# KC-decoder/Multimodal-Brain-Pattern-Identification_XAI

Measured on AMD Instinct MI355X. Metric: samples/sec train (multimodal SpectrogramCNN+EEGNet fusion, B=64/GPU, 4x128x256 spectro + 10000x19 EEG), higher is better.
Workload: dtype bf16

## Files before the change

include/brainxai.h:

```cpp
#ifndef BRAINXAI_H
#define BRAINXAI_H

#include <stddef.h>
#include <stdint.h>

#ifdef __cplusplus
extern "C" {
#endif

#define BX_VERSION 100

enum { BX_F32 = 0, BX_BF16 = 1 };
enum { BX_POOL_MAX = 0, BX_POOL_AVG = 1 };
enum { BX_OK = 0, BX_EINVAL = -1, BX_EDTYPE = -2, BX_EALIGN = -3, BX_EWORKSPACE = -4, BX_EHIP = -5,
       BX_EUNSUPPORTED = -6 };
enum { BX_ALGO_AUTO = 0, BX_ALGO_DIRECT = 1, BX_ALGO_MFMA = 2 };
enum { BX_EPI_RELU = 1, BX_EPI_MASK_BITS = 2 };

typedef void* bxStream;

int bx_version(void);
const char* bx_last_error_string(void);

int bx_nchw_to_nhwc(const float* src, void* dst, int B, int C, int H, int W, int Cp, int dtype, bxStream stream);
// ... 10 lines not shown
  void* packed_mfma;
  int Cout, Cin, I_p, O_p, transpose_flip, block_begin;
} bxPackJob;
int bx_conv3x3_pack_many(const bxPackJob* jobs_device, int njobs, int total_blocks, bxStream stream);
int bx_conv3x3_pack_many_layout(const bxPackJob* jobs_device, int njobs, int total_blocks, const float* src_nchw,
                                void* dst_nhwc_bf16, int B, int C, int H, int W, int Cp, bxStream stream);
int bx_conv3x3_pack_layout_ex(const bxPackJob* jobs_device, int njobs, int total_blocks, const float* src_nchw,
                              const float* const* src_slot, void* dst_nhwc_bf16, int B, int C, int H, int W, int Cp, bxStream stream);
int bx_conv3x3_pack_many_step(const bxPackJob* jobs_device, int njobs, int total_blocks, const float* src_nchw,
                              void* dst_nhwc_bf16, int B, int C, int H, int W, int Cp, uint64_t* state_a, uint64_t* out_a,
                              uint64_t* state_b, uint64_t* out_b, bxStream stream);
int bx_conv3x3_pair_supported(int C0_p, int C1, int C2, int dtype);
int bx_conv3x3_pair(const void* x, const void* packed1_mfma, const float* bias1, const void* packed2_mfma, const float* bias2,
                    void* y1, void* y2, unsigned char* mask1, unsigned char* mask2, int B, int H, int W, int C0_p, int C1, int C2,
                    int dtype, bxStream stream);
int bx_conv3x3(const void* x, const float* packed_f32, const void* packed_mfma, const float* bias,
               const void* relu_mask_src, const void* addend, void* y,
               int B, int H, int W, int Ci, int Co, int dtype, int flags, int algo, bxStream stream);
size_t bx_conv3x3_wgrad_workspace(int B, int H, int W, int Ci_p, int Co, int dtype, int algo);
int bx_conv3x3_wgrad(const void* x, const void* dz, float* dw_oihw, float* dbias, int B, int H, int W,
                     int Cin, int Ci_p, int Co, int dtype, int algo, void* workspace, size_t workspace_bytes,
                     bxStream stream);
typedef struct {
  const void* partial; float* dw; float* db;
  int nsplit, Cin, Co, ma, nb, ztiles, nfrag4, valid;
} bxWgradPending;
int bx_conv3x3_wgrad_chained(const void* x, const void* dz, float* dw_oihw, float* dbias, int B, int H, int W, int Cin,
                             int Ci_p, int Co, int dtype, int algo, void* workspace, size_t workspace_bytes,
                             bxWgradPending* pending, bxStream stream);
int bx_conv3x3_wgrad_finish(bxWgradPending* pending, bxStream stream);
int bx_conv3x3_carry(const void* x, const float* packed_f32, const void* packed_mfma, const float* bias,
                     const void* relu_mask_src, const void* addend, void* y, int B, int H, int W, int Ci, int Co,
                     int dtype, int flags, int algo, bxWgradPending* pending, bxStream stream);

int bx_profile_next_conv3(void* ev_start, void* ev_stop);

typedef struct {
  int B, H, W;
  int Cin_p;
  int C;
  int pool;
  int training;
  float eps, momentum;
  float dropout_p;
  uint32_t salt;
  int dtype;
  uint32_t* sync;
  void* route;
} bxTailDesc;
size_t bx_block_tail_route_bytes(const bxTailDesc* d);
#define BX_TAIL_SYNC_WORDS 8192
#define BX_TAIL_SYNC_FWD 0
#define BX_TAIL_SYNC_BWD 4096
size_t bx_block_tail_workspace(const bxTailDesc* d);
int bx_block_tail_fwd(const bxTailDesc* d, const void* y3, const void* x, const float* w1x1, int Cin,
                      const float* b1x1, const float* bn_weight, const float* bn_bias,
                      float* running_mean, float* running_var, int64_t* num_batches_tracked,
                      const uint64_t* seed, void* pooled, void* out, float* save_mean, float* save_invstd,
                      void* workspace, size_t workspace_bytes, bxStream stream);
int bx_set_tree_max_rows(int rows);
int bx_set_tail_fold(int mask);
int bx_block_conv3_tail_fwd(const bxTailDesc* d, const void* y2, const void* w3_mfma, const float* b3, void* y3,
                            const void* x, const float* w1x1, int Cin, const float* b1x1, const float* bn_weight,
                            const float* bn_bias, float* running_mean, float* running_var, int64_t* num_batches_tracked,
                            const uint64_t* seed, void* pooled, void* out, float* save_mean, float* save_invstd,
                            void* workspace, size_t workspace_bytes, bxStream stream);
// ... 171 lines not shown
```

multimodal-brain-pattern-identification_xai_amd/_lib.py:

```python
from __future__ import annotations

import ctypes as C
import os

HERE = os.path.dirname(os.path.abspath(__file__))
LIB_PATH = os.path.join(HERE, "libbrainxai.so")

BX_F32, BX_BF16 = 0, 1
BX_POOL_MAX, BX_POOL_AVG = 0, 1
BX_ALGO_AUTO, BX_ALGO_DIRECT, BX_ALGO_MFMA = 0, 1, 2
BX_EPI_RELU = 1
BX_EPI_MASK_BITS = 2
BX_TAIL_SYNC_WORDS = 8192
BX_EEG_CAM_CONV1, BX_EEG_CAM_DEPTHWISE, BX_EEG_CAM_SEPARABLE = 0, 1, 2

vp, i32, i64, u32, f32, sz = C.c_void_p, C.c_int, C.c_int64, C.c_uint32, C.c_float, C.c_size_t


class TailDesc(C.Structure):
    _fields_ = [("B", i32), ("H", i32), ("W", i32), ("Cin_p", i32), ("C", i32), ("pool", i32), ("training", i32),
                ("eps", f32), ("momentum", f32), ("dropout_p", f32), ("salt", u32), ("dtype", i32), ("sync", vp), ("route", vp)]


class EegDesc(C.Structure):
# ... 29 lines not shown
class PackJob(C.Structure):
    _fields_ = [("w_oihw", vp), ("packed_mfma", vp), ("Cout", i32), ("Cin", i32), ("I_p", i32), ("O_p", i32),
                ("transpose_flip", i32), ("block_begin", i32)]


class EegGrads(C.Structure):
    _fields_ = [(n, vp) for n in ("conv1_w", "bn1_w", "bn1_b", "dw_w", "bn2_w", "bn2_b", "sep_w", "bn3_w", "bn3_b")]


P = C.POINTER
SIGNATURES = {
    "bx_version": (i32, []),
    "bx_last_error_string": (C.c_char_p, []),
    "bx_nchw_to_nhwc": (i32, [vp, vp, i32, i32, i32, i32, i32, i32, vp]),
    "bx_nhwc_to_nchw": (i32, [vp, vp, i32, i32, i32, i32, i32, i32, vp]),
    "bx_conv3x3_pack": (i32, [vp, vp, vp, i32, i32, i32, i32, i32, vp]),
    "bx_conv3x3_packed_mfma_bytes": (sz, [i32, i32]),
    "bx_conv3x3_packed_split_bytes": (sz, [i32, i32]),
    "bx_conv3x3_pack_split": (i32, [vp, vp, i32, i32, i32, i32, i32, vp]),
    "bx_conv3x3_pack_many": (i32, [vp, i32, i32, vp]),
    "bx_conv3x3_pack_many_layout": (i32, [vp, i32, i32, vp, vp, i32, i32, i32, i32, i32, vp]),
    "bx_conv3x3_pack_layout_ex": (i32, [vp, i32, i32, vp, vp, vp, i32, i32, i32, i32, i32, vp]),
    "bx_conv3x3_pair_supported": (i32, [i32, i32, i32, i32]),
    "bx_conv3x3_pair": (i32, [vp] * 9 + [i32] * 7 + [vp]),
    "bx_conv3x3_pack_many_step": (i32, [vp, i32, i32, vp, vp, i32, i32, i32, i32, i32, vp, vp, vp, vp, vp]),
    "bx_scale_dev": (i32, [vp, vp, vp, sz, vp]),
    "bx_abs": (i32, [vp, vp, sz, vp]),
    "bx_conv3x3": (i32, [vp, vp, vp, vp, vp, vp, vp, i32, i32, i32, i32, i32, i32, i32, i32, vp]),
    "bx_conv3x3_carry": (i32, [vp, vp, vp, vp, vp, vp, vp, i32, i32, i32, i32, i32, i32, i32, i32, P(WgradPending), vp]),
    "bx_conv3x3_wgrad_workspace": (sz, [i32, i32, i32, i32, i32, i32, i32]),
    "bx_conv3x3_wgrad": (i32, [vp, vp, vp, vp, i32, i32, i32, i32, i32, i32, i32, i32, vp, sz, vp]),
    "bx_conv3x3_wgrad_chained": (i32, [vp, vp, vp, vp, i32, i32, i32, i32, i32, i32, i32, i32, vp, sz, P(WgradPending), vp]),
    "bx_conv3x3_wgrad_finish": (i32, [P(WgradPending), vp]),
    "bx_block_tail_workspace": (sz, [P(TailDesc)]),
    "bx_block_tail_fwd": (i32, [P(TailDesc), vp, vp, vp, i32, vp, vp, vp, vp, vp, vp, vp, vp, vp, vp, vp, vp, sz, vp]),
    "bx_set_tree_max_rows": (i32, [i32]),
    "bx_set_tail_fold": (i32, [i32]),
    "bx_block_tail_route_bytes": (sz, [vp]),
    "bx_block_conv3_tail_fwd": (i32, [P(TailDesc), vp, vp, vp, vp, vp, vp, i32, vp, vp, vp, vp, vp, vp, vp, vp, vp, vp, vp, vp, sz, vp]),
    "bx_block_tail_bwd": (i32, [P(TailDesc), vp, vp, vp, vp, vp, i32, vp, vp, vp, vp, vp, vp, vp, vp, vp, vp, vp, sz, vp]),
    "bx_relu": (i32, [vp, vp, sz, i32, vp]),
    "bx_gap_fc_lsm_fwd": (i32, [vp, vp, vp, vp, vp, i32, i32, i32, i32, i32, vp]),
    "bx_gap_fc_lsm_bwd": (i32, [vp, vp, vp, vp, vp, vp, vp, i32, i32, i32, i32, i32, vp]),
    "bx_linear_lsm_fwd": (i32, [vp, vp, vp, vp, i32, i32, i32, vp]),
    "bx_linear_lsm_bwd": (i32, [vp, vp, vp, vp, vp, vp, vp, i32, i32, i32, vp]),
    "bx_fusion_head_fwd": (i32, [vp, vp, vp, vp, vp, vp, vp, vp, i32, i32, i32, vp]),
    "bx_fusion_head_bwd": (i32, [vp] * 13 + [i32, i32, i32, vp]),
    "bx_mm_head_workspace": (sz, [i32, i32, i32]),
    "bx_mm_head_fwd": (i32, [vp] * 15 + [i32] * 7 + [vp]),
    "bx_mm_head_bwd": (i32, [vp] * 22 + [sz] + [i32] * 7 + [vp]),
    "bx_kldiv_fwd_bwd": (i32, [vp, vp, vp, vp, i32, i32, i32, f32, vp]),
    "bx_eeg_saved_bytes": (sz, [P(EegDesc)]),
    "bx_eeg_workspace": (sz, [P(EegDesc)]),
    "bx_eeg_features_fwd": (i32, [P(EegDesc), P(EegParams), vp, vp, vp, vp, vp, sz, vp]),
    "bx_eeg_features_bwd": (i32, [P(EegDesc), P(EegParams), vp, vp, vp, vp, P(EegGrads), vp, vp, sz, vp]),
    "bx_eeg_saved_layout": (i32, [P(EegDesc), P(sz), P(sz)]),
    "bx_eeg_gradcam_workspace": (sz, [P(EegDesc), i32, i32]),
    "bx_eeg_gradcam": (i32, [P(EegDesc), P(EegParams), vp, vp, vp, i32, i32, i32, vp, vp, vp, vp, sz, vp]),
    "bx_eeg_deep_saved_bytes": (sz, [P(EegDeepDesc)]),
    "bx_eeg_deep_workspace": (sz, [P(EegDeepDesc)]),
    "bx_eeg_deep_fwd": (i32, [P(EegDeepDesc), P(EegDeepParams), vp, vp, vp, vp, vp, vp, sz, vp]),
    "bx_eeg_deep_bwd": (i32, [P(EegDeepDesc), P(EegDeepParams), vp, vp, vp, vp, vp, P(EegDeepGrads), vp, vp, sz, vp]),
    "bx_attention_workspace": (sz, [i32]),
    "bx_attention_fwd": (i32, [vp] * 10 + [i32, i32, i32, vp]),
    "bx_attention_bwd": (i32, [vp] * 16 + [sz, i32, i32, i32, vp]),
    "bx_gradcam_reduce": (i32, [vp, vp, vp, vp, i32, i32, i32, i32, i32, i32, vp]),
# ... 58 lines not shown
```

multimodal-brain-pattern-identification_xai_amd/csrc/conv3x3_mfma.hip:

```cpp
#include <stdlib.h>
#include "bx_common.h"
#include <string.h>

typedef __attribute__((ext_vector_type(8))) short bf16x8;
typedef __attribute__((ext_vector_type(4))) float f32x4;
typedef unsigned int u32x4 __attribute__((ext_vector_type(4)));
typedef unsigned int u32x2 __attribute__((ext_vector_type(2)));

static inline int mfma_ck(int Ci) { return Ci < 64 ? Ci : 64; }
static inline int mfma_ks(int ck) { return (9 * ck + 31) / 32; }

int bx_conv3x3_mfma_supported(int Ci, int Co, int dtype) {
  if (dtype != BX_BF16) return 0;
  if (!(Ci == 8 || Ci == 16 || Ci == 32 || (Ci >= 64 && Ci % 64 == 0))) return 0;
  return (Co >= 16 && Co % 16 == 0) || (Co == 8 && (Ci == 16 || Ci == 32));
}
static inline int mfma_ow(int O_p) { return O_p < 16 ? 16 : O_p; }
extern "C" size_t bx_conv3x3_packed_mfma_bytes(int I_p, int O_p) {
  if (!bx_conv3x3_mfma_supported(I_p, O_p, BX_BF16)) return 0;
  const int ck = mfma_ck(I_p);
  return (size_t)(I_p / ck) * mfma_ks(ck) * mfma_ow(O_p) * 32 * sizeof(bf16_t);
}

__global__ void k_pack_mfma(const float* __restrict__ w, bf16_t* __restrict__ wp, int Cout, int Cin, int I_p, int O_p, int tf,
// ... 1416 lines not shown
      const float4 v3 = *reinterpret_cast<const float4*>(src + (size_t)(c + 3 * S) * per_split);
      s.x += v0.x; s.y += v0.y; s.z += v0.z; s.w += v0.w;
      s.x += v1.x; s.y += v1.y; s.z += v1.z; s.w += v1.w;
      s.x += v2.x; s.y += v2.y; s.z += v2.z; s.w += v2.w;
      s.x += v3.x; s.y += v3.y; s.z += v3.z; s.w += v3.w;
    }
    for (; c < nsplit; c += S) {
      const float4 v = *reinterpret_cast<const float4*>(src + (size_t)c * per_split);
      s.x += v.x; s.y += v.y; s.z += v.z; s.w += v.w;
    }
  }
  sm[threadIdx.x] = s;
  __syncthreads();
  if (part == 0 && live) {
    float4 r = sm[o];
    for (int k = 1; k < S; ++k) { const float4 v = sm[k * NO + o]; r.x += v.x; r.y += v.y; r.z += v.z; r.w += v.w; }
    const float rr[4] = {r.x, r.y, r.z, r.w};
    if (e4 < (size_t)nfrag4) {
      const int NT = 9 * MA * NB;
      const int lane = (int)(e4 & 63), tl = (int)(e4 >> 6);
      const int i = tl % NT, yz = tl / NT, z = yz % ztiles, y = yz / ztiles;
      const int n = i % NB, m = (i / NB) % MA, t = i / (NB * MA);
      const int cout = (z * NB + n) * 16 + (lane & 15), cin0 = (y * MA + m) * 16 + 4 * (lane >> 4);
#pragma unroll
      for (int j = 0; j < 4; ++j)
        if (cin0 + j < Cin) dw[((size_t)cout * Cin + cin0 + j) * 9 + t] = rr[j];
    } else if (db) {
      const size_t b0 = (e4 - nfrag4) * 4;
#pragma unroll
      for (int j = 0; j < 4; ++j) db[b0 + j] = rr[j];
    }
  }
}
__global__ __launch_bounds__(256) void k_wgrad_reduce3(WgradRedJob jb) {
  __shared__ float4 sm[256];
  wgrad_reduce3_body(jb, blockIdx.x, sm);
}

typedef __attribute__((ext_vector_type(4))) short s16x4;
typedef __attribute__((address_space(3))) s16x4 lds_s16x4;

__device__ __forceinline__ bf16x8 tr_read8(const char* lds, int off0, int off1) {
  const s16x4 lo = __builtin_amdgcn_ds_read_tr16_b64_v4i16((lds_s16x4*)(lds + off0));
  const s16x4 hi = __builtin_amdgcn_ds_read_tr16_b64_v4i16((lds_s16x4*)(lds + off1));
  return (bf16x8){lo[0], lo[1], lo[2], lo[3], hi[0], hi[1], hi[2], hi[3]};
}

template <int MA, int NB, int TW>
__global__ __launch_bounds__(256, 2) void k_wgrad_mfma(const bf16_t* __restrict__ x, const bf16_t* __restrict__ dz, float* __restrict__ partial,
    int H, int W, int Ci_p, int Co, int tiles_x, int tiles_y, int ntiles, int tiles_per_split, WgradRedJob prev, int zextra) {
  constexpr int TH = 8, HWID = TW + 2, HH = TH + 2, CIT = 16 * MA, COT = 16 * NB, XB = CIT * 2, ZB = COT * 2;
  constexpr int KPW = TH * TW / 32 / 4;
  constexpr int XS_BYTES = HH * HWID * XB;
  extern __shared__ __attribute__((aligned(16))) char lds[];
  if ((int)blockIdx.z < zextra) {
    const int rid = ((int)blockIdx.z * (int)gridDim.y + (int)blockIdx.y) * (int)gridDim.x + (int)blockIdx.x;
    if (rid < prev.nblocks) wgrad_reduce3_body(prev, rid, reinterpret_cast<float4*>(lds));
    return;
  }
  const int bz = (int)blockIdx.z - zextra, gz = (int)gridDim.z - zextra;
  char* xs = lds;
  char* zs = lds + XS_BYTES;
  const int wave = threadIdx.x >> 6, lane = threadIdx.x & 63, g = lane >> 4, li = lane & 15;
  const int q = li >> 2, pc = li & 3;
  const int ci0 = blockIdx.y * CIT, co0 = bz * COT;
  const bool want_bias = blockIdx.y == 0;

  f32x4 acc[9][MA][NB];
#pragma unroll
// ... 342 lines not shown
}
int bx_wgrad_mfma_supported(int Ci_p, int Co, int dtype) {
  return dtype == BX_BF16 && Ci_p % 8 == 0 && Co % 16 == 0 && (Co < 32 || Co % 32 == 0) && (Ci_p < 32 || Ci_p % 32 == 0);
}
size_t bx_wgrad_mfma_workspace(int B, int H, int W, int Ci_p, int Co) {
  const WgradPlan p = wgrad_plan(B, H, W, Ci_p, Co);
  return (size_t)p.nsplit * ((size_t)p.ytiles * p.ztiles * 9 * p.ma * p.nb * 256 + Co) * sizeof(float);
}
template <int MA, int NB, int TW>
static void launch_wgrad(const WgradPlan& p, const void* x, const void* dz, float* ws, int H, int W, int Ci_p, int Co, const WgradRedJob& prev,
                         int zextra, hipStream_t s) {
  dim3 grid(p.nsplit, p.ytiles, p.ztiles + zextra);
  hipLaunchKernelGGL((k_wgrad_mfma<MA, NB, TW>), grid, dim3(256), p.lds, s, (const bf16_t*)x, (const bf16_t*)dz, ws, H, W, Ci_p, Co,
                     p.tiles_x, p.tiles_y, p.ntiles, p.tps, prev, zextra);
}
static int wgrad_reduce_slices(size_t per_split, int nsplit, bool chained) {
  if (!chained) return per_split >= 65536 ? 4 : per_split >= 8192 ? 16 : 64;
  int S = 1;
  while (S < 64 && nsplit > 8 * S) S *= 2;
  return S;
}
static WgradRedJob wgrad_job_from(const bxWgradPending* pd, bool chained) {
  WgradRedJob jb;
  jb.partial = (const float*)pd->partial; jb.dw = pd->dw; jb.db = pd->db; jb.nsplit = pd->nsplit; jb.Cin = pd->Cin; jb.Co = pd->Co;
  jb.MA = pd->ma; jb.NB = pd->nb; jb.ztiles = pd->ztiles; jb.nfrag4 = pd->nfrag4;
  const size_t per_split = (size_t)pd->nfrag4 * 4 + pd->Co;
  jb.S = wgrad_reduce_slices(per_split, pd->nsplit, chained);
  const int per_wg = 256 / jb.S;
  jb.nblocks = (int)((per_split / 4 + per_wg - 1) / per_wg);
  return jb;
}
int bx_wgrad_mfma_finish(bxWgradPending* pd, hipStream_t s) {
  if (!pd || !pd->valid) return BX_OK;
  const WgradRedJob jb = wgrad_job_from(pd, false);
  hipLaunchKernelGGL(k_wgrad_reduce3, dim3(jb.nblocks), dim3(256), 0, s, jb);
  pd->valid = 0;
  BX_CHECK_LAUNCH("bx_conv3x3_wgrad(mfma reduce)");
  return BX_OK;
}
int bx_wgrad_mfma_launch(const void* x, const void* dz, float* dw, float* db, int B, int H, int W, int Cin, int Ci_p,
                         int Co, void* ws, size_t ws_bytes, bxWgradPending* pending, hipStream_t s) {
  const WgradPlan p = wgrad_plan(B, H, W, Ci_p, Co);
  (void)ws_bytes;
  BX_REQUIRE((size_t)B * H * W * (Ci_p > Co ? Ci_p : Co) * 2 < ((size_t)1 << 31), "bx_conv3x3_wgrad(mfma): an activation tensor of 2 GiB or more is not supported");
  BX_REQUIRE(!pending || !pending->valid || pending->partial != ws, "bx_conv3x3_wgrad(chained): the pending partials live in this call's workspace");
  float* part = (float*)ws;
  WgradRedJob prev;
  memset(&prev, 0, sizeof(prev));
  int zextra = 0;
  if (pending && pending->valid) {
    prev = wgrad_job_from(pending, true);
    zextra = (prev.nblocks + p.nsplit * p.ytiles - 1) / (p.nsplit * p.ytiles);
  }
  if (p.ma == 2 && p.nb == 2) {
    const int nred = pending && pending->valid ? (prev.nblocks + 7) / 8 * 8 : 0;
    const int ranges8 = (p.nsplit + 7) / 8;
    const int nwg = nred + ranges8 * 8 * p.ytiles * p.ztiles;
    const size_t lds = (size_t)10 * (p.tw + 2) * 64 + (size_t)8 * p.tw * 64 + 256;
    if (p.tw == 16)
      hipLaunchKernelGGL((k_wgrad_own<16, 2>), dim3(nwg), dim3(256), lds, s, (const bf16_t*)x, (const bf16_t*)dz, part, H, W, Ci_p, Co,
                         p.tiles_x, p.tiles_y, p.ntiles, p.tps, p.nsplit, p.ytiles, p.ztiles, prev, nred);
    else
      hipLaunchKernelGGL((k_wgrad_own<32, 2>), dim3(nwg), dim3(256), lds, s, (const bf16_t*)x, (const bf16_t*)dz, part, H, W, Ci_p, Co,
                         p.tiles_x, p.tiles_y, p.ntiles, p.tps, p.nsplit, p.ytiles, p.ztiles, prev, nred);
  } else {
#define BX_WG(MA_, NB_) do { if (p.tw == 16) launch_wgrad<MA_, NB_, 16>(p, x, dz, part, H, W, Ci_p, Co, prev, zextra, s); \
                             else launch_wgrad<MA_, NB_, 32>(p, x, dz, part, H, W, Ci_p, Co, prev, zextra, s); } while (0)
    if (p.ma == 1 && p.nb == 1) BX_WG(1, 1);
    else if (p.ma == 1) BX_WG(1, 2);
    else BX_WG(2, 1);
#undef BX_WG
  }
  BX_CHECK_LAUNCH("bx_conv3x3_wgrad(mfma)");
  bxWgradPending cur;
  cur.partial = part; cur.dw = dw; cur.db = db; cur.nsplit = p.nsplit; cur.Cin = Cin; cur.Co = Co; cur.ma = p.ma; cur.nb = p.nb;
  cur.ztiles = p.ztiles; cur.nfrag4 = p.ytiles * p.ztiles * 9 * p.ma * p.nb * 64; cur.valid = 1;
  if (pending) { *pending = cur; return BX_OK; }
  return bx_wgrad_mfma_finish(&cur, s);
}
```

multimodal-brain-pattern-identification_xai_amd/ops.py:

```python
from __future__ import annotations

import ctypes as C
from types import SimpleNamespace

import torch

from . import _lib as L

CONV_ALGO = L.BX_ALGO_AUTO
WGRAD_ALGO = L.BX_ALGO_AUTO
CONV_PROFILE = None
import os as _os
OVERLAP_EEG = int(_os.environ.get("BX_OVERLAP_EEG", "1"))
OVERLAP_EEG_DDP = _os.environ.get("BX_OVERLAP_EEG_DDP", "0") == "1"


def overlap_eeg_now() -> bool:
    if CONV_PROFILE is not None or not (OVERLAP_EEG >= 2 or (OVERLAP_EEG == 1 and torch.cuda.is_current_stream_capturing())):
        return False
    import torch.distributed as dist
    return OVERLAP_EEG_DDP or not (dist.is_available() and dist.is_initialized())


def fork_eeg(device, *read_on_side):
# ... 405 lines not shown
def _wgrad(x, dz, w: torch.Tensor, b: torch.Tensor, chain: bool = False):
    lib = L.load()
    B, H, W, Cip = x.shape
    Co = dz.shape[3]
    dt = bx_dtype(x.dtype)
    algo = WGRAD_ALGO
    need = lib.bx_conv3x3_wgrad_workspace(B, H, W, Cip, Co, dt, algo)
    dw, db = new_grad(w), new_grad(b)
    if chain and WGRAD_CHAIN and algo != L.BX_ALGO_DIRECT:
        st = _wg_chain_state(x.device)
        if st.pend.valid and st.stream != _stream():
            wgrad_flush(x.device)
        buf = st.ring[st.slot]
        if buf is None or buf.numel() < need:
            if buf is not None:
                st.retired.append(buf)
            big = max([int(need), 1 << 20] + [b.numel() for b in st.ring if b is not None])
            buf = torch.empty(big, dtype=torch.uint8, device=x.device)
            st.ring[st.slot] = buf
        st.stream = _stream()
        with _Timed("wgrad", ("conv", B, H, W, Cip, Co)):
            L.check(lib.bx_conv3x3_wgrad_chained(_p(x), _p(dz), _p(dw), _p(db), B, H, W, w.shape[1], Cip, Co, dt, algo, _p(buf), buf.numel(),
                                                 C.byref(st.pend), st.stream), "bx_conv3x3_wgrad_chained")
        st.keep = (buf, dw, db)
        st.slot ^= 1
        return dw, db
    ws = workspace(need, x.device)
    with _Timed("wgrad", ("conv", B, H, W, Cip, Co)):
        L.check(lib.bx_conv3x3_wgrad(_p(x), _p(dz), _p(dw), _p(db), B, H, W, w.shape[1], Cip, Co, dt, algo, _p(ws), ws.numel(), _stream()),
                "bx_conv3x3_wgrad")
    return dw, db


def _tail_desc(x, shape, dt, cfg, route=None) -> L.TailDesc:
    B, H, W, Cc = shape
    return L.TailDesc(B, H, W, x.shape[3], Cc, L.BX_POOL_MAX if cfg.pool == "max" else L.BX_POOL_AVG, 1 if cfg.training else 0,
                      cfg.eps, cfg.momentum, float(cfg.dropout_p), cfg.salt, bx_dtype(dt), _p(cfg.sync), _p(route))


class BlockFn(torch.autograd.Function):

    @staticmethod
    def forward(ctx, x, w1, b1, w2, b2, w3, b3, bnw, bnb, w11, b11, rm, rv, nbt, cfg):
        lib = L.load()
        dt = x.dtype
        ws_, bs_ = (w1, w2, w3), (b1, b2, b3)
        acts, pre = [x], None
        B, H, W, _ = x.shape
        Cc = w3.shape[0]
        fused = FUSE_POOL and dt == torch.bfloat16 and CONV_ALGO != L.BX_ALGO_DIRECT and cfg.preact != 3 and Cc >= 16
        packed3 = None
        first = 0
        masks = None
        if (CONV_PAIR and dt == torch.bfloat16 and CONV_ALGO != L.BX_ALGO_DIRECT and cfg.preact not in (1, 2)
                and lib.bx_conv3x3_pair_supported(x.shape[3], w1.shape[0], w2.shape[0], bx_dtype(dt))):
            pk = []
            for k in range(2):
                packed = cfg.prepacked.get(cfg.pack_base + k, False) if cfg.prepacked is not None else None
                pk.append(packed if packed is not None else _pack(ws_[k], flip=False, dtype=dt))
            if pk[0][1] is not None and pk[1][1] is not None:
                need_y1 = cfg.keep is not None or (getattr(cfg, "grad_mode", True) and any(ctx.needs_input_grad[:11]))
                y1 = torch.empty(B, H, W, w1.shape[0], dtype=dt, device=x.device) if need_y1 else None
                y2 = torch.empty(B, H, W, w2.shape[0], dtype=dt, device=x.device)
                if need_y1 and MASK_BITS and w1.shape[0] <= 32:
                    masks = (torch.empty(B, H, W, w1.shape[0] // 4, dtype=torch.uint8, device=x.device),
                             torch.empty(B, H, W, w2.shape[0] // 4, dtype=torch.uint8, device=x.device))
                with _Timed("fwd", ("pair", B, H, W, x.shape[3], (w1.shape[0], w2.shape[0]))):
                    L.check(lib.bx_conv3x3_pair(_p(x), _p(pk[0][1]), _p(b1), _p(pk[1][1]), _p(b2), _p(y1), _p(y2),
                                                _p(masks[0]) if masks else None, _p(masks[1]) if masks else None, B, H, W, x.shape[3],
                                                w1.shape[0], w2.shape[0], bx_dtype(dt), _stream()), "bx_conv3x3_pair")
                acts += [y1 if y1 is not None else x.new_empty(0), y2]
                first = 2
        for k in range(first, 3):
            packed = cfg.prepacked.get(cfg.pack_base + k, False) if cfg.prepacked is not None else None
            if packed is None:
                packed = _pack(ws_[k], flip=False, dtype=dt)
            if k == 2 and fused and packed[1] is not None:
                packed3 = packed
                break
            if cfg.preact == k + 1:
                pre = _conv(acts[-1], packed, bs_[k], None, None, False, dt)
                y = torch.empty_like(pre)
                L.check(lib.bx_relu(_p(pre), _p(y), pre.numel(), bx_dtype(dt), _stream()), "bx_relu")
            else:
                y = _conv(acts[-1], packed, bs_[k], None, None, True, dt)
            acts.append(y)
        seed = None
        if cfg.training and cfg.dropout_p > 0:
            seed = cfg.seed if cfg.seed is not None else next_seed(x.device)
        pooled = torch.empty(B, H // 2, W // 2, Cc, dtype=dt, device=x.device)
        out = torch.empty_like(pooled)
        mean = torch.empty(Cc, dtype=torch.float32, device=x.device)
        invstd = torch.empty_like(mean)
        route = None
        if packed3 is not None:
            need_bwd = getattr(cfg, "grad_mode", True) and any(ctx.needs_input_grad[:11])
            use_route = TAIL_ROUTE and cfg.keep is None
            y3 = torch.empty(B, H, W, Cc, dtype=dt, device=x.device) if (cfg.keep is not None or (need_bwd and not use_route)) else None
            if need_bwd and use_route:
                route = torch.empty(B * (H // 2) * (W // 2) * Cc // 2, dtype=torch.uint8, device=x.device)
            desc = _tail_desc(x, (B, H, W, Cc), dt, cfg, route)
            ws = workspace(lib.bx_block_tail_workspace(C.byref(desc)), x.device)
            if CONV_PROFILE is not None:
                pe0, pe1 = torch.cuda.Event(enable_timing=True), torch.cuda.Event(enable_timing=True)
                pe0.record(); pe1.record()
                L.check(lib.bx_profile_next_conv3(pe0.cuda_event, pe1.cuda_event), "bx_profile_next_conv3")
                CONV_PROFILE.append(("fwd", pe0, pe1, ("conv3+pool", B, H, W, acts[2].shape[3], Cc)))
            L.check(lib.bx_block_conv3_tail_fwd(C.byref(desc), _p(acts[2]), _p(packed3[1]), _p(b3), _p(y3), _p(x), _p(w11), w11.shape[1], _p(b11),
                                                _p(bnw), _p(bnb), _p(rm), _p(rv), _p(nbt), _p(seed), _p(pooled), _p(out), _p(mean), _p(invstd),
                                                _p(ws), ws.numel(), _stream()), "bx_block_conv3_tail_fwd")
            acts.append(y3)
        else:
            y3 = acts[3]
            desc = _tail_desc(x, tuple(y3.shape), dt, cfg)
            ws = workspace(lib.bx_block_tail_workspace(C.byref(desc)), x.device)
            L.check(lib.bx_block_tail_fwd(C.byref(desc), _p(y3), _p(x), _p(w11), w11.shape[1], _p(b11), _p(bnw), _p(bnb), _p(rm), _p(rv), _p(nbt),
                                          _p(seed), _p(pooled), _p(out), _p(mean), _p(invstd), _p(ws), ws.numel(), _stream()), "bx_block_tail_fwd")
        ctx.cfg, ctx.desc, ctx.seed = cfg, desc, seed
        ctx.masks = masks
        ctx.route, ctx.y3_shape = route, (B, H, W, Cc)
        ctx.save_for_backward(x, acts[1], acts[2], y3 if y3 is not None else x.new_empty(0), pooled, mean, invstd, w1, b1, w2, b2, w3, b3,
                              bnw, bnb, w11, b11)
        if pre is not None:
            cfg.capture["act"] = pre
        if cfg.keep is not None:
            cfg.keep["acts"] = (acts[1], acts[2], y3)
        return out

    @staticmethod
    def backward(ctx, dout):
        lib = L.load()
        x, y1, y2, y3, pooled, mean, invstd, w1, b1, w2, b2, w3, b3, bnw, bnb, w11, b11 = ctx.saved_tensors
        cfg, desc, seed = ctx.cfg, ctx.desc, ctx.seed
        dt = x.dtype
        need_dx = ctx.needs_input_grad[0]
        need_w = any(ctx.needs_input_grad[1:11])
        dout = dout.contiguous()
        dz3 = torch.empty(ctx.y3_shape, dtype=dt, device=x.device)
        if y3.numel() == 0:
            y3 = None
        dx_skip = torch.empty_like(x) if need_dx else None
        need_bn = ctx.needs_input_grad[7] or ctx.needs_input_grad[8]
        d_bnw, d_bnb = (new_grad(bnw), new_grad(bnb)) if need_bn else (torch.empty_like(bnw), torch.empty_like(bnb))
        d_w11, d_b11 = (new_grad(w11), new_grad(b11)) if need_w else (None, None)
        ws = workspace(lib.bx_block_tail_workspace(C.byref(desc)), x.device)
        L.check(lib.bx_block_tail_bwd(C.byref(desc), _p(dout), _p(y3), _p(x), _p(pooled), _p(w11), w11.shape[1], _p(bnw), _p(mean), _p(invstd),
                                      _p(seed), _p(dz3), _p(dx_skip), _p(d_bnw), _p(d_bnb), _p(d_w11), _p(d_b11), _p(ws), ws.numel(), _stream()),
                "bx_block_tail_bwd")
        if cfg.preact == 3:
            cfg.capture["grad"] = dz3
        acts = (x, y1, y2)
        wts = (w1, w2, w3)
        bss = (b1, b2, b3)
        grads_w, grads_b = [None] * 3, [None] * 3
        dz = dz3
        for k in (2, 1, 0):
            if need_w:
                grads_w[k], grads_b[k] = _wgrad(acts[k], dz, wts[k], bss[k], chain=True)
            packed = cfg.prepacked.get(cfg.pack_base + k, True) if cfg.prepacked is not None else None
            if k > 0:
                mb = ctx.masks is not None and CONV_ALGO != L.BX_ALGO_DIRECT
                dz = _conv(dz, packed or _pack(wts[k], flip=True, dtype=dt), None, ctx.masks[k - 1] if mb else acts[k], None, False, dt,
                           mask_bits=mb)
                if cfg.preact == k:
                    cfg.capture["grad"] = dz
            elif need_dx:
                dz = _conv(dz, packed or _pack(wts[0], flip=True, dtype=dt), None, None, dx_skip, False, dt, carry=need_w)
        if need_w:
            wgrad_flush(x.device)
        dx = dz if need_dx else None
        if not need_bn:
            d_bnw = d_bnb = None
        return (dx, grads_w[0], grads_b[0], grads_w[1], grads_b[1], grads_w[2], grads_b[2], d_bnw, d_bnb, d_w11, d_b11,
                None, None, None, None)


class GapFcLsmFn(torch.autograd.Function):

    @staticmethod
    def forward(ctx, feat, w, b):
        B, H, W, Cc = feat.shape
        N = w.shape[0]
        gap = torch.empty(B, Cc, dtype=torch.float32, device=feat.device)
        logp = torch.empty(B, N, dtype=torch.float32, device=feat.device)
        L.check(L.load().bx_gap_fc_lsm_fwd(_p(feat), _p(w), _p(b), _p(gap), _p(logp), B, H * W, Cc, N, bx_dtype(feat.dtype), _stream()),
                "bx_gap_fc_lsm_fwd")
        ctx.shape, ctx.dt = (B, H, W, Cc), feat.dtype
        ctx.save_for_backward(gap, logp, w, b)
        return logp
# ... 302 lines not shown
```

Baseline: 46390.

## Fuse stage-1 conv backward dgrad and wgrad into one MFMA kernel

Adds a fused backward kernel for 16->16 3x3 conv layers that computes the data gradient (with ReLU masking from the saved activation) and the weight gradient in a single tile pass. Each tile is loaded into LDS once and reused by both. For the last pair it also computes conv1's weight gradient from the in-LDS data gradient, so that gradient never goes to global memory. The previous layer's pending wgrad reduction is folded into the same launch as extra blocks, and the two final reductions share one launch. In exchange it drops the mask-bit path for these blocks and uses a larger LDS footprint, which may lower occupancy.

```diff
diff --git a/include/brainxai.h b/include/brainxai.h
--- a/include/brainxai.h
+++ b/include/brainxai.h
@@ -66,6 +66,10 @@
 int bx_conv3x3_carry(const void* x, const float* packed_f32, const void* packed_mfma, const float* bias,
                      const void* relu_mask_src, const void* addend, void* y, int B, int H, int W, int Ci, int Co,
                      int dtype, int flags, int algo, bxWgradPending* pending, bxStream stream);
+size_t bx_conv3x3_bwd_fused_workspace(int B, int H, int W, int with_w1);
+int bx_conv3x3_bwd_fused(const void* dz, const void* xl, const void* packed_flip, void* dzo, const void* x0, float* dw, float* db,
+                         float* dw0, float* db0, int B, int H, int W, int Cin0, void* workspace, size_t workspace_bytes,
+                         bxWgradPending* pending, bxStream stream);
 
 int bx_profile_next_conv3(void* ev_start, void* ev_stop);
 
diff --git a/multimodal-brain-pattern-identification_xai_amd/_lib.py b/multimodal-brain-pattern-identification_xai_amd/_lib.py
--- a/multimodal-brain-pattern-identification_xai_amd/_lib.py
+++ b/multimodal-brain-pattern-identification_xai_amd/_lib.py
@@ -85,6 +85,8 @@
     "bx_conv3x3_wgrad": (i32, [vp, vp, vp, vp, i32, i32, i32, i32, i32, i32, i32, i32, vp, sz, vp]),
     "bx_conv3x3_wgrad_chained": (i32, [vp, vp, vp, vp, i32, i32, i32, i32, i32, i32, i32, i32, vp, sz, P(WgradPending), vp]),
     "bx_conv3x3_wgrad_finish": (i32, [P(WgradPending), vp]),
+    "bx_conv3x3_bwd_fused_workspace": (sz, [i32, i32, i32, i32]),
+    "bx_conv3x3_bwd_fused": (i32, [vp] * 9 + [i32] * 4 + [vp, sz, P(WgradPending), vp]),
     "bx_block_tail_workspace": (sz, [P(TailDesc)]),
     "bx_block_tail_fwd": (i32, [P(TailDesc), vp, vp, vp, i32, vp, vp, vp, vp, vp, vp, vp, vp, vp, vp, vp, vp, sz, vp]),
     "bx_set_tree_max_rows": (i32, [i32]),
diff --git a/multimodal-brain-pattern-identification_xai_amd/csrc/conv3x3_mfma.hip b/multimodal-brain-pattern-identification_xai_amd/csrc/conv3x3_mfma.hip
--- a/multimodal-brain-pattern-identification_xai_amd/csrc/conv3x3_mfma.hip
+++ b/multimodal-brain-pattern-identification_xai_amd/csrc/conv3x3_mfma.hip
@@ -1472,9 +1472,10 @@
     }
   }
 }
-__global__ __launch_bounds__(256) void k_wgrad_reduce3(WgradRedJob jb) {
+__global__ __launch_bounds__(256) void k_wgrad_reduce3(WgradRedJob jb, WgradRedJob jb2) {
   __shared__ float4 sm[256];
-  wgrad_reduce3_body(jb, blockIdx.x, sm);
+  if ((int)blockIdx.x < jb.nblocks) wgrad_reduce3_body(jb, blockIdx.x, sm);
+  else wgrad_reduce3_body(jb2, (int)blockIdx.x - jb.nblocks, sm);
 }
 
 typedef __attribute__((ext_vector_type(4))) short s16x4;
@@ -1883,8 +1884,8 @@
 }
 int bx_wgrad_mfma_finish(bxWgradPending* pd, hipStream_t s) {
   if (!pd || !pd->valid) return BX_OK;
-  const WgradRedJob jb = wgrad_job_from(pd, false);
-  hipLaunchKernelGGL(k_wgrad_reduce3, dim3(jb.nblocks), dim3(256), 0, s, jb);
+  const WgradRedJob jb = wgrad_job_from(pd, false), none = {};
+  hipLaunchKernelGGL(k_wgrad_reduce3, dim3(jb.nblocks), dim3(256), 0, s, jb, none);
   pd->valid = 0;
   BX_CHECK_LAUNCH("bx_conv3x3_wgrad(mfma reduce)");
   return BX_OK;
@@ -1929,3 +1930,270 @@
   if (pending) { *pending = cur; return BX_OK; }
   return bx_wgrad_mfma_finish(&cur, s);
 }
+
+__device__ __forceinline__ void wgrad_store_1x1(f32x4 (&acc)[9], float bsum, float* __restrict__ out, char* lds) {
+  const int wave = threadIdx.x >> 6, lane = threadIdx.x & 63;
+  constexpr int NT = 9, SLOTS = 3;
+  float4* red4 = reinterpret_cast<float4*>(lds);
+  __syncthreads();
+#pragma unroll
+  for (int s = 1; s < 4; ++s) {
+    const int dst = (wave + s) & 3, src = (wave - s) & 3;
+#pragma unroll
+    for (int i = 0; i < NT; ++i)
+      if ((i & 3) == dst) red4[(wave * SLOTS + i / 4) * 64 + lane] = make_float4(acc[i][0], acc[i][1], acc[i][2], acc[i][3]);
+    __syncthreads();
+#pragma unroll
+    for (int i = 0; i < NT; ++i)
+      if ((i & 3) == wave) {
+        const float4 v = red4[(src * SLOTS + i / 4) * 64 + lane];
+        acc[i][0] += v.x; acc[i][1] += v.y; acc[i][2] += v.z; acc[i][3] += v.w;
+      }
+    __syncthreads();
+  }
+  float4* out4 = reinterpret_cast<float4*>(out);
+#pragma unroll
+  for (int i = 0; i < NT; ++i)
+    if ((i & 3) == wave) out4[i * 64 + lane] = make_float4(acc[i][0], acc[i][1], acc[i][2], acc[i][3]);
+  float* red = reinterpret_cast<float*>(lds);
+  float v = bsum;
+  v += __shfl_xor(v, 16, 64);
+  v += __shfl_xor(v, 32, 64);
+  if (lane < 16) red[wave * 16 + lane] = v;
+  __syncthreads();
+  if (threadIdx.x < 16) out[NT * 256 + threadIdx.x] = red[threadIdx.x] + red[16 + threadIdx.x] + red[32 + threadIdx.x] + red[48 + threadIdx.x];
+}
+
+template <bool W1>
+__global__ __launch_bounds__(256, 2) void k_conv_mfma_bwd(const bf16_t* __restrict__ dz, const bf16_t* __restrict__ xl, const bf16_t* __restrict__ wp,
+    const bf16_t* __restrict__ x0, bf16_t* __restrict__ dzo, float* __restrict__ partial, int H, int W, int tiles_x, int tiles_y, int ntiles,
+    int tps, int nsplit, uint32_t act_bytes, WgradRedJob red, int nred) {
+  constexpr int TH = 8, TW = 32, HWID = TW + 2, HH = TH + 2, PB = 32, KS = 5, MP = TH * TW / 64, TPR = TW / 16;
+  constexpr int NU = HH * HWID * 2, NR = (NU + 255) / 256;
+  constexpr int NU0 = HH * HWID, NR0 = (NU0 + 255) / 256;
+  constexpr int IMG = HH * HWID * PB;
+  constexpr int PER_SPLIT = 9 * 256 + 16;
+  extern __shared__ __attribute__((aligned(16))) char lds[];
+  if ((int)blockIdx.x < nred) {
+    if ((int)blockIdx.x < red.nblocks) wgrad_reduce3_body(red, (int)blockIdx.x, reinterpret_cast<float4*>(lds));
+    return;
+  }
+  const int split = (int)blockIdx.x - nred;
+  char* zs = lds;
+  char* xs = lds + IMG;
+  char* x0s = lds + 2 * IMG;
+  char* d1s = lds + 3 * IMG;
+  const int wave = threadIdx.x >> 6, lane = threadIdx.x & 63, g = lane >> 4, li = lane & 15;
+  const int q = li >> 2, pc = li & 3;
+  const __amdgpu_buffer_rsrc_t zres = __builtin_amdgcn_make_buffer_rsrc((void*)dz, 0, act_bytes, 0x00020000);
+  const __amdgpu_buffer_rsrc_t xres = __builtin_amdgcn_make_buffer_rsrc((void*)xl, 0, act_bytes, 0x00020000);
+  const __amdgpu_buffer_rsrc_t x0res = __builtin_amdgcn_make_buffer_rsrc((void*)(W1 ? x0 : xl), 0, W1 ? act_bytes / 2 : 0u, 0x00020000);
+  const __amdgpu_buffer_rsrc_t yres = __builtin_amdgcn_make_buffer_rsrc((void*)(W1 ? xl : dzo), 0, W1 ? 0u : act_bytes, 0x00020000);
+  int hpy[NR], hpx[NR];
+  uint32_t hrel[NR];
+#pragma unroll
+  for (int k = 0; k < NR; ++k) {
+    const int u = threadIdx.x + k * 256;
+    const int p = u / 2, c = u % 2;
+    hpy[k] = u < NU ? p / HWID - 1 : -100000;
+    hpx[k] = p % HWID - 1;
+    hrel[k] = (uint32_t)(((p / HWID - 1) * W + (p % HWID - 1)) * 16 + c * 8) * 2u;
+  }
+  int h0y[NR0], h0x[NR0];
+  uint32_t h0rel[NR0];
+#pragma unroll
+  for (int k = 0; k < NR0; ++k) {
+    const int p = threadIdx.x + k * 256;
+    h0y[k] = p < NU0 ? p / HWID - 1 : -100000;
+    h0x[k] = p % HWID - 1;
+    h0rel[k] = (uint32_t)(((p / HWID - 1) * W + (p % HWID - 1)) * 8) * 2u;
+  }
+  uint4 rz[NR], rx[NR], r0[W1 ? NR0 : 1];
+  auto fetch = [&](int tile) {
+    const int tx = tile % tiles_x, ty = (tile / tiles_x) % tiles_y, b = tile / (tiles_x * tiles_y);
+    const int y0 = ty * TH, xo = tx * TW;
+    const uint32_t pix0 = (uint32_t)((b * H + y0) * W + xo);
+#pragma unroll
+    for (int k = 0; k < NR; ++k) {
+      const bool ok = (unsigned)(y0 + hpy[k]) < (unsigned)H && (unsigned)(xo + hpx[k]) < (unsigned)W;
+      const uint32_t off = ok ? pix0 * 32u + hrel[k] : 0x80000000u;
+      const u32x4 v = __builtin_amdgcn_raw_buffer_load_b128(zres, off, 0, 0);
+      const u32x4 w = __builtin_amdgcn_raw_buffer_load_b128(xres, off, 0, 0);
+      rz[k] = make_uint4(v.x, v.y, v.z, v.w);
+      rx[k] = make_uint4(w.x, w.y, w.z, w.w);
+    }
+    if constexpr (W1) {
+#pragma unroll
+      for (int k = 0; k < NR0; ++k) {
+        const bool ok = (unsigned)(y0 + h0y[k]) < (unsigned)H && (unsigned)(xo + h0x[k]) < (unsigned)W;
+        const u32x4 v = __builtin_amdgcn_raw_buffer_load_b128(x0res, ok ? pix0 * 16u + h0rel[k] : 0x80000000u, 0, 0);
+        r0[k] = make_uint4(v.x, v.y, v.z, v.w);
+      }
+    }
+  };
+  if constexpr (W1) {
+    for (int p = threadIdx.x; p < NU0; p += 256) *reinterpret_cast<uint4*>(x0s + p * PB + 16) = make_uint4(0u, 0u, 0u, 0u);
+  }
+  f32x4 aw[9], aw1[W1 ? 9 : 1];
+#pragma unroll
+  for (int t = 0; t < 9; ++t) aw[t] = (f32x4){0.f, 0.f, 0.f, 0.f};
+#pragma unroll
+  for (int t = 0; t < (W1 ? 9 : 1); ++t) aw1[t] = (f32x4){0.f, 0.f, 0.f, 0.f};
+  float bsum = 0.f, bsum1 = 0.f;
+  const int t_begin = split * tps;
+  const int t_end = t_begin + tps < ntiles ? t_begin + tps : ntiles;
+  if (t_begin < t_end) fetch(t_begin);
+  for (int tile = t_begin; tile < t_end; ++tile) {
+    const int tx = tile % tiles_x, ty = (tile / tiles_x) % tiles_y, b = tile / (tiles_x * tiles_y);
+    const int y0 = ty * TH, xo = tx * TW;
+    __syncthreads();
+#pragma unroll
+    for (int k = 0; k < NR; ++k) {
+      const int u = threadIdx.x + k * 256;
+      if (u < NU) {
+        *reinterpret_cast<uint4*>(zs + u * 16) = rz[k];
+        *reinterpret_cast<uint4*>(xs + u * 16) = rx[k];
+      }
+    }
+    if constexpr (W1) {
+#pragma unroll
+      for (int k = 0; k < NR0; ++k) {
+        const int p = threadIdx.x + k * 256;
+        if (p < NU0) *reinterpret_cast<uint4*>(x0s + p * PB) = r0[k];
+      }
+    }
+    __syncthreads();
+    if (tile + 1 < t_end) fetch(tile + 1);
+    f32x4 acc[MP];
+#pragma unroll
+    for (int i = 0; i < MP; ++i) acc[i] = (f32x4){0.f, 0.f, 0.f, 0.f};
+    bf16x8 a[3];
+    auto load_a = [&](int s, bf16x8& dst) { dst = *reinterpret_cast<const bf16x8*>(wp + ((size_t)s * 16 + li) * 32 + 8 * g); };
+    load_a(0, a[0]);
+    load_a(1, a[1]);
+#pragma unroll
+    for (int s = 0; s < KS; ++s) {
+      if (s + 2 < KS) load_a(s + 2, a[(s + 2) % 3]);
+      __builtin_amdgcn_sched_barrier(0);
+      const int q0 = s * 32 + 8 * g;
+      int tap = q0 / 16;
+      const int c = (q0 % 16) / 8;
+      const bool valid = tap < 9;
+      if (!valid) tap = 0;
+      const int dy = tap / 3, dx = tap - 3 * dy;
+#pragma unroll
+      for (int i = 0; i < MP; ++i) {
+        const int t = wave * MP + i;
+        const int p = (t / TPR + dy) * HWID + (t % TPR) * 16 + li + dx;
+        bf16x8 bv = *reinterpret_cast<const bf16x8*>(zs + p * PB + 16 * c);
+        if (!valid) bv = (bf16x8){0, 0, 0, 0, 0, 0, 0, 0};
+        acc[i] = __builtin_amdgcn_mfma_f32_16x16x32_bf16(a[s % 3], bv, acc[i], 0, 0, 0);
+      }
+    }
+#pragma unroll
+    for (int i = 0; i < MP; ++i) {
+      const int t = wave * MP + i;
+      const int r = t / TPR, col = (t % TPR) * 16 + li;
+      const u32x2 m = *reinterpret_cast<const u32x2*>(xs + ((r + 1) * HWID + col + 1) * PB + 8 * g);
+      const uint32_t mm[4] = {m.x & 0xffffu, m.x >> 16, m.y & 0xffffu, m.y >> 16};
+      float v[4] = {acc[i][0] + 0.f, acc[i][1] + 0.f, acc[i][2] + 0.f, acc[i][3] + 0.f};
+#pragma unroll
+      for (int j = 0; j < 4; ++j) v[j] = (mm[j] != 0u && mm[j] < 0x8000u) ? v[j] : 0.f;
+      const u32x2 out = {pack2bf(v[0], v[1]), pack2bf(v[2], v[3])};
+      if constexpr (W1) {
+        *reinterpret_cast<u32x2*>(d1s + (r * TW + col) * PB + 8 * g) = out;
+      } else {
+        const bool inb = y0 + r < H && xo + col < W;
+        const uint32_t off = inb ? (uint32_t)((((b * H + y0 + r) * W + xo + col) * 16 + 4 * g) * 2) : 0x80000000u;
+        __builtin_amdgcn_raw_buffer_store_b64(out, yres, off, 0, 0);
+      }
+    }
+#pragma unroll
+    for (int ks = 0; ks < 2; ++ks) {
+      __builtin_amdgcn_sched_barrier(0);
+      const int row = wave * 2 + ks;
+      const int col0 = 8 * g + q, col1 = 8 * g + 4 + q;
+      const bf16x8 bfr = tr_read8(zs, ((row + 1) * HWID + col0 + 1) * PB + 8 * pc, ((row + 1) * HWID + col1 + 1) * PB + 8 * pc);
+#pragma unroll
+      for (int j = 0; j < 8; ++j) bsum += __uint_as_float(((uint32_t)(unsigned short)bfr[j]) << 16);
+#pragma unroll
+      for (int tap = 0; tap < 9; ++tap) {
+        const int dy = tap / 3, dx = tap % 3;
+        const bf16x8 afr = tr_read8(xs, ((row + dy) * HWID + col0 + dx) * PB + 8 * pc, ((row + dy) * HWID + col1 + dx) * PB + 8 * pc);
+        aw[tap] = __builtin_amdgcn_mfma_f32_16x16x32_bf16(afr, bfr, aw[tap], 0, 0, 0);
+      }
+      if constexpr (W1) {
+        __builtin_amdgcn_sched_barrier(0);
+        const bf16x8 bf1 = tr_read8(d1s, (row * TW + col0) * PB + 8 * pc, (row * TW + col1) * PB + 8 * pc);
+#pragma unroll
+        for (int j = 0; j < 8; ++j) bsum1 += __uint_as_float(((uint32_t)(unsigned short)bf1[j]) << 16);
+#pragma unroll
+        for (int tap = 0; tap < 9; ++tap) {
+          const int dy = tap / 3, dx = tap % 3;
+          const bf16x8 afr = tr_read8(x0s, ((row + dy) * HWID + col0 + dx) * PB + 8 * pc, ((row + dy) * HWID + col1 + dx) * PB + 8 * pc);
+          aw1[tap] = __builtin_amdgcn_mfma_f32_16x16x32_bf16(afr, bf1, aw1[tap], 0, 0, 0);
+        }
+      }
+    }
+  }
+  wgrad_store_1x1(aw, bsum, partial + (size_t)split * PER_SPLIT, lds);
+  if constexpr (W1) wgrad_store_1x1(aw1, bsum1, partial + ((size_t)nsplit + split) * PER_SPLIT, lds);
+}
+
+struct FusedBwdPlan { int tiles_x, tiles_y, ntiles, tps, nsplit; };
+static FusedBwdPlan fused_bwd_plan(int B, int H, int W) {
+  FusedBwdPlan p;
+  p.tiles_x = (W + 31) / 32; p.tiles_y = (H + 7) / 8; p.ntiles = p.tiles_x * p.tiles_y * B;
+  constexpr int want_wgs = 512;
+  const int want = want_wgs < p.ntiles ? want_wgs : p.ntiles;
+  p.tps = (p.ntiles + want - 1) / want;
+  p.nsplit = (p.ntiles + p.tps - 1) / p.tps;
+  return p;
+}
+extern "C" size_t bx_conv3x3_bwd_fused_workspace(int B, int H, int W, int with_w1) {
+  const FusedBwdPlan p = fused_bwd_plan(B, H, W);
+  return (size_t)p.nsplit * (9 * 256 + 16) * sizeof(float) * (with_w1 ? 2 : 1);
+}
+extern "C" int bx_conv3x3_bwd_fused(const void* dz, const void* xl, const void* packed_flip, void* dzo, const void* x0, float* dw, float* db,
+                                    float* dw0, float* db0, int B, int H, int W, int Cin0, void* ws, size_t ws_bytes, bxWgradPending* pending,
+                                    bxStream stream) {
+  hipStream_t s = (hipStream_t)stream;
+  const bool w1 = x0 != nullptr;
+  BX_REQUIRE(dz && xl && packed_flip && dw && db && ws && B > 0 && H > 0 && W > 0, "bx_conv3x3_bwd_fused: bad arguments");
+  BX_REQUIRE(w1 ? (!dzo && dw0 && db0 && Cin0 > 0 && Cin0 <= 8) : (dzo && !dw0 && !db0),
+             "bx_conv3x3_bwd_fused: either dzo (data gradient stored) or x0 with dw0 / db0 (conv1's weight gradient, 1..8 input channels)");
+  BX_REQUIRE((size_t)B * H * W * 16 * 2 < ((size_t)1 << 31), "bx_conv3x3_bwd_fused: an activation tensor of 2 GiB or more is not supported");
+  const FusedBwdPlan p = fused_bwd_plan(B, H, W);
+  const size_t need = bx_conv3x3_bwd_fused_workspace(B, H, W, w1);
+  BX_REQUIRE(ws_bytes >= need, "bx_conv3x3_bwd_fused: workspace %zu < %zu", ws_bytes, need);
+  BX_REQUIRE(!pending || !pending->valid || pending->partial != ws, "bx_conv3x3_bwd_fused: the pending partials live in this call's workspace");
+  WgradRedJob prev = {};
+  int nred = 0;
+  if (pending && pending->valid) { prev = wgrad_job_from(pending, true); nred = prev.nblocks; pending->valid = 0; }
+  constexpr int IMG = 10 * 34 * 32;
+  const size_t lds = w1 ? (size_t)3 * IMG + 8 * 32 * 32 : (size_t)2 * IMG;
+  const uint32_t act_bytes = (uint32_t)((size_t)B * H * W * 16 * 2);
+  float* part = (float*)ws;
+  if (w1)
+    hipLaunchKernelGGL((k_conv_mfma_bwd<true>), dim3((unsigned)(p.nsplit + nred)), dim3(256), lds, s, (const bf16_t*)dz, (const bf16_t*)xl,
+                       (const bf16_t*)packed_flip, (const bf16_t*)x0, (bf16_t*)nullptr, part, H, W, p.tiles_x, p.tiles_y, p.ntiles, p.tps, p.nsplit,
+                       act_bytes, prev, nred);
+  else
+    hipLaunchKernelGGL((k_conv_mfma_bwd<false>), dim3((unsigned)(p.nsplit + nred)), dim3(256), lds, s, (const bf16_t*)dz, (const bf16_t*)xl,
+                       (const bf16_t*)packed_flip, (const bf16_t*)nullptr, (bf16_t*)dzo, part, H, W, p.tiles_x, p.tiles_y, p.ntiles, p.tps, p.nsplit,
+                       act_bytes, prev, nred);
+  BX_CHECK_LAUNCH("bx_conv3x3_bwd_fused");
+  bxWgradPending cur = {};
+  cur.partial = part; cur.dw = dw; cur.db = db; cur.nsplit = p.nsplit; cur.Cin = 16; cur.Co = 16; cur.ma = 1; cur.nb = 1;
+  cur.ztiles = 1; cur.nfrag4 = 9 * 64; cur.valid = 1;
+  if (!w1) {
+    if (pending) { *pending = cur; return BX_OK; }
+    return bx_wgrad_mfma_finish(&cur, s);
+  }
+  bxWgradPending cur0 = cur;
+  cur0.partial = part + (size_t)p.nsplit * (9 * 256 + 16); cur0.dw = dw0; cur0.db = db0; cur0.Cin = Cin0;
+  const WgradRedJob j1 = wgrad_job_from(&cur, false), j0 = wgrad_job_from(&cur0, false);
+  hipLaunchKernelGGL(k_wgrad_reduce3, dim3((unsigned)(j1.nblocks + j0.nblocks)), dim3(256), 0, s, j1, j0);
+  BX_CHECK_LAUNCH("bx_conv3x3_bwd_fused(reduce)");
+  return BX_OK;
+}
diff --git a/multimodal-brain-pattern-identification_xai_amd/ops.py b/multimodal-brain-pattern-identification_xai_amd/ops.py
--- a/multimodal-brain-pattern-identification_xai_amd/ops.py
+++ b/multimodal-brain-pattern-identification_xai_amd/ops.py
@@ -461,6 +461,37 @@
     return dw, db
 
 
+def _bwd_fused(dz, xl, packed, w, b, x0, w0, b0):
+    lib = L.load()
+    B, H, W, _ = dz.shape
+    st = _wg_chain_state(dz.device)
+    if st.pend.valid and st.stream != _stream():
+        wgrad_flush(dz.device)
+    need = lib.bx_conv3x3_bwd_fused_workspace(B, H, W, 1 if x0 is not None else 0)
+    buf = st.ring[st.slot]
+    if buf is None or buf.numel() < need:
+        if buf is not None:
+            st.retired.append(buf)
+        big = max([int(need), 1 << 20] + [t.numel() for t in st.ring if t is not None])
+        buf = torch.empty(big, dtype=torch.uint8, device=dz.device)
+        st.ring[st.slot] = buf
+    st.stream = _stream()
+    dw, db = new_grad(w), new_grad(b)
+    dw0, db0 = (new_grad(w0), new_grad(b0)) if x0 is not None else (None, None)
+    dzo = torch.empty_like(dz) if x0 is None else None
+    if packed[1] is None or packed[4] != "bf16":
+        raise RuntimeError("brainxai: the fused stage-1 backward needs the bf16 MFMA data-gradient operand")
+    with _Timed("dgrad", ("conv", B, H, W, 16, 16)):
+        L.check(lib.bx_conv3x3_bwd_fused(_p(dz), _p(xl), _p(packed[1]), _p(dzo), _p(x0), _p(dw), _p(db), _p(dw0), _p(db0), B, H, W,
+                                         w0.shape[1], _p(buf), buf.numel(), C.byref(st.pend), st.stream), "bx_conv3x3_bwd_fused")
+    if x0 is None:
+        st.keep = (buf, dw, db)
+        st.slot ^= 1
+    else:
+        st.keep = None
+    return dw, db, dzo, (dw0, db0)
+
+
 def _tail_desc(x, shape, dt, cfg, route=None) -> L.TailDesc:
     B, H, W, Cc = shape
     return L.TailDesc(B, H, W, x.shape[3], Cc, L.BX_POOL_MAX if cfg.pool == "max" else L.BX_POOL_AVG, 1 if cfg.training else 0,
@@ -481,6 +512,7 @@
         packed3 = None
         first = 0
         masks = None
+        fuse_bwd = False
         if (CONV_PAIR and dt == torch.bfloat16 and CONV_ALGO != L.BX_ALGO_DIRECT and cfg.preact not in (1, 2)
                 and lib.bx_conv3x3_pair_supported(x.shape[3], w1.shape[0], w2.shape[0], bx_dtype(dt))):
             pk = []
@@ -491,7 +523,9 @@
                 need_y1 = cfg.keep is not None or (getattr(cfg, "grad_mode", True) and any(ctx.needs_input_grad[:11]))
                 y1 = torch.empty(B, H, W, w1.shape[0], dtype=dt, device=x.device) if need_y1 else None
                 y2 = torch.empty(B, H, W, w2.shape[0], dtype=dt, device=x.device)
-                if need_y1 and MASK_BITS and w1.shape[0] <= 32:
+                fuse_bwd = (need_y1 and cfg.keep is None and WGRAD_ALGO != L.BX_ALGO_DIRECT and x.shape[3] == 8
+                            and tuple(w2.shape[:2]) == (16, 16) and tuple(w3.shape[:2]) == (16, 16) and any(ctx.needs_input_grad[1:11]))
+                if need_y1 and MASK_BITS and w1.shape[0] <= 32 and not fuse_bwd:
                     masks = (torch.empty(B, H, W, w1.shape[0] // 4, dtype=torch.uint8, device=x.device),
                              torch.empty(B, H, W, w2.shape[0] // 4, dtype=torch.uint8, device=x.device))
                 with _Timed("fwd", ("pair", B, H, W, x.shape[3], (w1.shape[0], w2.shape[0]))):
@@ -547,6 +581,7 @@
                                           _p(seed), _p(pooled), _p(out), _p(mean), _p(invstd), _p(ws), ws.numel(), _stream()), "bx_block_tail_fwd")
         ctx.cfg, ctx.desc, ctx.seed = cfg, desc, seed
         ctx.masks = masks
+        ctx.fuse_bwd = fuse_bwd
         ctx.route, ctx.y3_shape = route, (B, H, W, Cc)
         ctx.save_for_backward(x, acts[1], acts[2], y3 if y3 is not None else x.new_empty(0), pooled, mean, invstd, w1, b1, w2, b2, w3, b3,
                               bnw, bnb, w11, b11)
@@ -583,7 +618,17 @@
         bss = (b1, b2, b3)
         grads_w, grads_b = [None] * 3, [None] * 3
         dz = dz3
-        for k in (2, 1, 0):
+        layers = (2, 1, 0)
+        if ctx.fuse_bwd and need_w:
+            for k in (2, 1):
+                packed = cfg.prepacked.get(cfg.pack_base + k, True) if cfg.prepacked is not None else None
+                w1_form = k == 1 and not need_dx
+                grads_w[k], grads_b[k], dz, g0 = _bwd_fused(dz, acts[k], packed or _pack(wts[k], flip=True, dtype=dt), wts[k], bss[k],
+                                                            x if w1_form else None, w1, b1)
+            if w1_form:
+                grads_w[0], grads_b[0] = g0
+            layers = () if w1_form else (0,)
+        for k in layers:
             if need_w:
                 grads_w[k], grads_b[k] = _wgrad(acts[k], dz, wts[k], bss[k], chain=True)
             packed = cfg.prepacked.get(cfg.pack_base + k, True) if cfg.prepacked is not None else None
```

Result: faster. 48090 (median of 6 runs) (+3.7%).
